# daniabib/ComfyUI_ProPainter_Nodes

Hardware: NVIDIA H100
Metric: inpainted frames/sec at 640x360, 80-frame subvideo (higher is better)
Workload: dtype f16

## Files before the change

### comfyui_propainter_nodes_b200/csrc/conv_epilogue.cuh

```cuda
#pragma once
#include "conv_igemm.cuh"
#include "wgmma_ops.cuh"

namespace ppconv {

template <int ACT, bool ACC = false>
__device__ __forceinline__ void act16_t(float (&v)[16], float slope) {
#pragma unroll
  for (int i = 0; i < 16; ++i) {
    if (ACT == PP_ACT_RELU) v[i] = fmaxf(v[i], 0.f);
    else if (ACT == PP_ACT_LRELU) v[i] = v[i] > 0.f ? v[i] : v[i] * slope;
    else if (ACT == PP_ACT_SIGMOID) v[i] = ppx::sigmoidf_(v[i]);
    else if (ACT == PP_ACT_TANH) v[i] = ACC ? ppx::tanh_acc(v[i]) : tanhf(v[i]);
    else if (ACT == PP_ACT_GELU) v[i] = ppx::gelu_erf(v[i]);
  }
}
template <bool ACC = false>
__device__ __forceinline__ void act16(float (&v)[16], int act, float slope) {
  switch (act) {
    case PP_ACT_RELU: act16_t<PP_ACT_RELU, ACC>(v, slope); break;
    case PP_ACT_LRELU: act16_t<PP_ACT_LRELU, ACC>(v, slope); break;
    case PP_ACT_SIGMOID: act16_t<PP_ACT_SIGMOID, ACC>(v, slope); break;
    case PP_ACT_TANH: act16_t<PP_ACT_TANH, ACC>(v, slope); break;
    case PP_ACT_GELU: act16_t<PP_ACT_GELU, ACC>(v, slope); break;
    default: break;
  }
}

__device__ __forceinline__ void load16(const __half* src, int nvalid, bool vec, float (&r)[16]) {
  if (vec && nvalid == 16) {
    const uint4 a = reinterpret_cast<const uint4*>(src)[0], b = reinterpret_cast<const uint4*>(src)[1];
    const __half2* ha = reinterpret_cast<const __half2*>(&a);
    const __half2* hb = reinterpret_cast<const __half2*>(&b);
#pragma unroll
    for (int i = 0; i < 4; ++i) {
      const float2 fa = __half22float2(ha[i]), fb = __half22float2(hb[i]);
      r[2 * i] = fa.x; r[2 * i + 1] = fa.y; r[8 + 2 * i] = fb.x; r[8 + 2 * i + 1] = fb.y;
    }
  } else {
#pragma unroll
    for (int i = 0; i < 16; ++i) r[i] = i < nvalid ? __half2float(src[i]) : 0.f;
  }
}
__device__ __forceinline__ void store16(__half* dst, int nvalid, bool vec, const float (&v)[16]) {
  if (vec && nvalid == 16) {
    __align__(16) __half2 h[8];
#pragma unroll
    for (int i = 0; i < 8; ++i) h[i] = __floats2half2_rn(v[2 * i], v[2 * i + 1]);
    reinterpret_cast<uint4*>(dst)[0] = reinterpret_cast<uint4*>(h)[0];
    reinterpret_cast<uint4*>(dst)[1] = reinterpret_cast<uint4*>(h)[1];
  } else {
#pragma unroll
    for (int i = 0; i < 16; ++i)
      if (i < nvalid) dst[i] = __float2half_rn(v[i]);
  }
}

__device__ __forceinline__ void unpack16(const uint4& a, const uint4& b, float (&r)[16]) {
  const __half2* ha = reinterpret_cast<const __half2*>(&a);
  const __half2* hb = reinterpret_cast<const __half2*>(&b);
#pragma unroll
  for (int i = 0; i < 4; ++i) {
    const float2 fa = __half22float2(ha[i]), fb = __half22float2(hb[i]);
    r[2 * i] = fa.x; r[2 * i + 1] = fa.y; r[8 + 2 * i] = fb.x; r[8 + 2 * i + 1] = fb.y;
  }
}

struct EpiAux {
  uint4 a0[2], a1[2];
  bool have;
};
__device__ __forceinline__ void conv_epilogue_prefetch16(const PPConvParams& p, long long mrow, int ng0, int epi, bool vec,
                                                         EpiAux& x) {
  x.have = false;
  if (!vec || p.Cout_g - ng0 < 16) return;
  const __half* s0 = nullptr;
  const __half* s1 = nullptr;
  if (epi == PP_EPI_STD) {
    if (p.aux0 != nullptr) s0 = p.aux0 + mrow * p.aux0_cstride + p.aux0_coff + ng0;
  } else if (epi == PP_EPI_GRU_ZR) {
    const int half_c = p.Cout_g >> 1;
    if (ng0 >= half_c) s0 = p.aux0 + mrow * p.aux0_cstride + p.aux0_coff + (ng0 - half_c);
  } else {
    s0 = p.aux0 + mrow * p.aux0_cstride + p.aux0_coff + ng0;
    s1 = p.aux1 + mrow * p.aux1_cstride + p.aux1_coff + ng0;
  }
  if (s0 == nullptr) return;
  x.have = true;
  x.a0[0] = reinterpret_cast<const uint4*>(s0)[0];
  x.a0[1] = reinterpret_cast<const uint4*>(s0)[1];
  if (s1 != nullptr) {
    x.a1[0] = reinterpret_cast<const uint4*>(s1)[0];
    x.a1[1] = reinterpret_cast<const uint4*>(s1)[1];
  }
}

__device__ __forceinline__ void conv_epilogue16(const PPConvParams& p, const uint32_t (&raw)[16], long long mrow, int g,
                                                int ng0, int epi, bool vec, const EpiAux* pre = nullptr,
                                                uint4* sm0 = nullptr, uint4* sm1 = nullptr) {
    const int nvalid = min(16, p.Cout_g - ng0);
    float v[16];
#pragma unroll
    for (int i = 0; i < 16; ++i) v[i] = __uint_as_float(raw[i]);
    if (p.bias != nullptr) {
      const float* bp = p.bias + g * p.Cout_g + ng0;
      if (vec && nvalid == 16) {
#pragma unroll
        for (int i = 0; i < 4; ++i) {
          const float4 b4 = __ldg(reinterpret_cast<const float4*>(bp) + i);
          v[4 * i] += b4.x; v[4 * i + 1] += b4.y; v[4 * i + 2] += b4.z; v[4 * i + 3] += b4.w;
        }
      } else {
#pragma unroll
        for (int i = 0; i < 16; ++i)
          if (i < nvalid) v[i] += __ldg(bp + i);
      }
    }
    if (epi == PP_EPI_STD) {
      act16(v, p.act1, p.slope);
      if (p.scale != 1.f) {
#pragma unroll
        for (int i = 0; i < 16; ++i) v[i] *= p.scale;
      }
      if (p.aux0 != nullptr) {
        float r[16];
        if (pre != nullptr && pre->have) unpack16(pre->a0[0], pre->a0[1], r);
        else load16(p.aux0 + mrow * p.aux0_cstride + p.aux0_coff + ng0, nvalid, vec, r);
#pragma unroll
        for (int i = 0; i < 16; ++i) v[i] += r[i];
      }
      act16(v, p.act2, p.slope);
      const long long o = mrow * p.out_cstride + p.out_coff + (long long)g * p.out_gstep + ng0;
      if (p.out_fp32) {
        float* dst = reinterpret_cast<float*>(p.out) + o;
        if (vec && nvalid == 16) {
#pragma unroll
          for (int i = 0; i < 4; ++i)
            reinterpret_cast<float4*>(dst)[i] = make_float4(v[4 * i], v[4 * i + 1], v[4 * i + 2], v[4 * i + 3]);
        } else {
#pragma unroll
          for (int i = 0; i < 16; ++i)
            if (i < nvalid) dst[i] = v[i];
        }
      } else if (sm0 != nullptr) {
        __align__(16) __half2 h[8];
#pragma unroll
        for (int i = 0; i < 8; ++i) h[i] = __floats2half2_rn(v[2 * i], v[2 * i + 1]);
        *sm0 = reinterpret_cast<uint4*>(h)[0];
        *sm1 = reinterpret_cast<uint4*>(h)[1];
      } else {
        store16(reinterpret_cast<__half*>(p.out) + o, nvalid, vec, v);
      }
    } else if (epi == PP_EPI_GRU_ZR) {
      const int half_c = p.Cout_g >> 1;
      act16_t<PP_ACT_SIGMOID>(v, 0.f);
      if (ng0 < half_c) {
        store16(reinterpret_cast<__half*>(p.out) + mrow * p.out_cstride + p.out_coff + ng0, nvalid, vec, v);
      } else {
        const int c = ng0 - half_c;
        float h[16];
        if (pre != nullptr && pre->have) unpack16(pre->a0[0], pre->a0[1], h);
        else load16(p.aux0 + mrow * p.aux0_cstride + p.aux0_coff + c, nvalid, vec, h);
#pragma unroll
        for (int i = 0; i < 16; ++i) v[i] *= h[i];
        store16(p.out2 + mrow * p.out2_cstride + p.out2_coff + c, nvalid, vec, v);
      }
    } else {
      float h[16], z[16];
      if (pre != nullptr && pre->have) {
        unpack16(pre->a0[0], pre->a0[1], h);
        unpack16(pre->a1[0], pre->a1[1], z);
      } else {
        load16(p.aux0 + mrow * p.aux0_cstride + p.aux0_coff + ng0, nvalid, vec, h);
        load16(p.aux1 + mrow * p.aux1_cstride + p.aux1_coff + ng0, nvalid, vec, z);
      }
      act16_t<PP_ACT_TANH>(v, 0.f);
#pragma unroll
      for (int i = 0; i < 16; ++i) v[i] = (1.f - z[i]) * h[i] + z[i] * v[i];
      store16(reinterpret_cast<__half*>(p.out) + mrow * p.out_cstride + p.out_coff + ng0, nvalid, vec, v);
    }
}

__device__ __forceinline__ float tf32_rna(float x) {
  uint32_t r;
  asm("cvt.rna.tf32.f32 %0, %1;" : "=r"(r) : "f"(x));
  return __uint_as_float(r);
}
__device__ __forceinline__ void load16_split(const float* src, int lo, int nvalid, bool vec, float (&r)[16]) {
  if (vec && nvalid == 16) {
#pragma unroll
    for (int i = 0; i < 4; ++i) {
      const float4 h = reinterpret_cast<const float4*>(src)[i], l = reinterpret_cast<const float4*>(src + lo)[i];
      r[4 * i] = h.x + l.x; r[4 * i + 1] = h.y + l.y; r[4 * i + 2] = h.z + l.z; r[4 * i + 3] = h.w + l.w;
    }
  } else {
#pragma unroll
    for (int i = 0; i < 16; ++i) r[i] = i < nvalid ? src[i] + src[lo + i] : 0.f;
  }
}
__device__ __forceinline__ void store16_split(float* dst, int lo, int nvalid, bool vec, const float (&v)[16]) {
  float h[16], l[16];
#pragma unroll
  for (int i = 0; i < 16; ++i) { h[i] = tf32_rna(v[i]); l[i] = v[i] - h[i]; }
  if (vec && nvalid == 16) {
#pragma unroll
    for (int i = 0; i < 4; ++i) {
      reinterpret_cast<float4*>(dst)[i] = make_float4(h[4 * i], h[4 * i + 1], h[4 * i + 2], h[4 * i + 3]);
      reinterpret_cast<float4*>(dst + lo)[i] = make_float4(l[4 * i], l[4 * i + 1], l[4 * i + 2], l[4 * i + 3]);
    }
  } else {
#pragma unroll
    for (int i = 0; i < 16; ++i)
      if (i < nvalid) { dst[i] = h[i]; dst[lo + i] = l[i]; }
  }
}

__device__ __forceinline__ void conv_epilogue16_split(const PPConvParams& p, const float (&acc)[16], long long mrow, int g,
                                                      int ng0, bool vec) {
  const int nvalid = min(16, p.Cout_g - ng0);
  float v[16];
#pragma unroll
  for (int i = 0; i < 16; ++i) v[i] = acc[i];
  if (p.bias != nullptr) {
    const float* bp = p.bias + g * p.Cout_g + ng0;
#pragma unroll
    for (int i = 0; i < 16; ++i)
      if (i < nvalid) v[i] += __ldg(bp + i);
  }
  const float* aux0 = reinterpret_cast<const float*>(p.aux0);
  const float* aux1 = reinterpret_cast<const float*>(p.aux1);
  float* out = reinterpret_cast<float*>(p.out);
  if (p.epi == PP_EPI_STD) {
    act16<true>(v, p.act1, p.slope);
    if (p.scale != 1.f) {
#pragma unroll
      for (int i = 0; i < 16; ++i) v[i] *= p.scale;
    }
    if (aux0 != nullptr) {
      float r[16];
      load16_split(aux0 + mrow * p.aux0_cstride + p.aux0_coff + ng0, p.aux0_lo, nvalid, vec, r);
#pragma unroll
      for (int i = 0; i < 16; ++i) v[i] += r[i];
    }
    act16<true>(v, p.act2, p.slope);
    float* dst = out + mrow * p.out_cstride + p.out_coff + (long long)g * p.out_gstep + ng0;
    if (p.out_fp32) {
      if (vec && nvalid == 16) {
#pragma unroll
        for (int i = 0; i < 4; ++i)
          reinterpret_cast<float4*>(dst)[i] = make_float4(v[4 * i], v[4 * i + 1], v[4 * i + 2], v[4 * i + 3]);
      } else {
#pragma unroll
        for (int i = 0; i < 16; ++i)
          if (i < nvalid) dst[i] = v[i];
      }
    } else {
      store16_split(dst, p.out_lo, nvalid, vec, v);
    }
  } else if (p.epi == PP_EPI_GRU_ZR) {
    const int half_c = p.Cout_g >> 1;
    act16_t<PP_ACT_SIGMOID, true>(v, 0.f);
    if (ng0 < half_c) {
      store16_split(out + mrow * p.out_cstride + p.out_coff + ng0, p.out_lo, nvalid, vec, v);
    } else {
      const int c = ng0 - half_c;
      float h[16];
      load16_split(aux0 + mrow * p.aux0_cstride + p.aux0_coff + c, p.aux0_lo, nvalid, vec, h);
#pragma unroll
      for (int i = 0; i < 16; ++i) v[i] *= h[i];
      store16_split(reinterpret_cast<float*>(p.out2) + mrow * p.out2_cstride + p.out2_coff + c, p.out2_lo, nvalid, vec, v);
    }
  } else {
    float h[16], z[16];
    load16_split(aux0 + mrow * p.aux0_cstride + p.aux0_coff + ng0, p.aux0_lo, nvalid, vec, h);
    load16_split(aux1 + mrow * p.aux1_cstride + p.aux1_coff + ng0, p.aux1_lo, nvalid, vec, z);
    act16_t<PP_ACT_TANH, true>(v, 0.f);
#pragma unroll
    for (int i = 0; i < 16; ++i) v[i] = (1.f - z[i]) * h[i] + z[i] * v[i];
    store16_split(out + mrow * p.out_cstride + p.out_coff + ng0, p.out_lo, nvalid, vec, v);
  }
}

constexpr int STG_LD = 40;
constexpr int STG_BYTES = 64 * STG_LD * 4;

template <int N, class Emit>
__device__ __forceinline__ void drain_acc(const float (&acc)[N / 2], float* stg, int t128, int bar_id, Emit&& emit) {
  const int wrow = 16 * (t128 >> 5) + ((t128 & 31) >> 2), wcol = 2 * (t128 & 3);
#pragma unroll 1
  for (int c0 = 0; c0 < N; c0 += 32) {
#pragma unroll
    for (int cc = 0; cc < N; cc += 32) {
      if (cc == c0) {
#pragma unroll
        for (int j = 0; j < 4; ++j) {
          if (cc + 8 * j < N) {
            const int i = (cc / 8 + j) * 4;
            *reinterpret_cast<float2*>(stg + wrow * STG_LD + 8 * j + wcol) = make_float2(acc[i], acc[i + 1]);
            *reinterpret_cast<float2*>(stg + (wrow + 8) * STG_LD + 8 * j + wcol) = make_float2(acc[i + 2], acc[i + 3]);
          }
        }
      }
    }
    ppx::named_bar(bar_id, 128);
    const int c = c0 + 16 * (t128 & 1);
    if (c < N) emit(stg + (t128 >> 1) * STG_LD + 16 * (t128 & 1), t128 >> 1, c);
    ppx::named_bar(bar_id, 128);
  }
}

template <bool SPLIT = false>
__device__ __forceinline__ void epilogue_from_stage(const PPConvParams& p, const float* src, long long mrow, int g, int ng0,
                                                    uint4* sm0, uint4* sm1) {
  if constexpr (SPLIT) {
    float acc[16];
#pragma unroll
    for (int i = 0; i < 16; i += 4) {
      const float4 v = *reinterpret_cast<const float4*>(src + i);
      acc[i] = v.x; acc[i + 1] = v.y; acc[i + 2] = v.z; acc[i + 3] = v.w;
    }
    conv_epilogue16_split(p, acc, mrow, g, ng0, p.vec_ok != 0);
  } else {
    uint32_t raw[16];
#pragma unroll
    for (int i = 0; i < 16; i += 4) {
      const float4 v = *reinterpret_cast<const float4*>(src + i);
      raw[i] = __float_as_uint(v.x); raw[i + 1] = __float_as_uint(v.y);
      raw[i + 2] = __float_as_uint(v.z); raw[i + 3] = __float_as_uint(v.w);
    }
    conv_epilogue16(p, raw, mrow, g, ng0, p.epi, p.vec_ok != 0, nullptr, sm0, sm1);
  }
}

template <int V>
struct IntC { static constexpr int value = V; };
template <int MAX_N, class F>
__device__ __forceinline__ void with_tile_width(int bn, F&& f) {
  switch (bn) {
    case 16: f(IntC<16>{}); break;
    case 32: f(IntC<32>{}); break;
    case 48: f(IntC<48>{}); break;
    case 64: f(IntC<64>{}); break;
    case 80: f(IntC<80>{}); break;
    case 96: f(IntC<96>{}); break;
    case 112: f(IntC<112>{}); break;
    case 128: f(IntC<128>{}); break;
    default:
      if constexpr (MAX_N > 128) {
        switch (bn) {
          case 144: f(IntC<144>{}); break;
          case 160: f(IntC<160>{}); break;
          case 176: f(IntC<176>{}); break;
          case 192: f(IntC<192>{}); break;
          case 208: f(IntC<208>{}); break;
          case 224: f(IntC<224>{}); break;
          case 240: f(IntC<240>{}); break;
          case 256: f(IntC<256>{}); break;
          default: __trap();
        }
      } else {
        __trap();
      }
  }
}

}
```

### comfyui_propainter_nodes_b200/csrc/conv_halo.cu

```cuda
#include <cuda.h>
#include <stdlib.h>
#include <string.h>

#include <memory>

#include "conv_epilogue.cuh"
#include "conv_igemm.cuh"
#include "dcn_sample.cuh"

namespace {

constexpr int NUM_THREADS = 384;
constexpr int NUM_EPI_THREADS = 256;
constexpr int WARP_A = 8, WARP_B = 9;
constexpr int MAX_SA = 4, MAX_SB = 8;
constexpr int SMEM_BUDGET = 186 * 1024;

struct HaloParams {
  PPConvParams c;
  CUtensorMap tmap[PP_MAX_SEGS];
  int MT;
  int BW, BH;
  int tiles_x, tiles_y, n_tiles;
  int a_stage_bytes, b_stage_bytes, SA, SB;
  int tps;
  int chunks;
  int flat;
  int n_img;
  int sub_bytes;
  int debug;
  int tstore;
  int out_stage_bytes;
  CUtensorMap tmap_out;
};

__device__ __forceinline__ void tma_load_4d(uint32_t dst, const void* tmap, int c0, int c1, int c2, int c3, uint64_t* bar) {
  asm volatile(
      "cp.async.bulk.tensor.4d.shared::cluster.global.mbarrier::complete_tx::bytes [%0], [%1, {%3, %4, %5, %6}], [%2];" ::"r"(dst),
      "l"(tmap), "r"(ppx::smem_u32(bar)), "r"(c0), "r"(c1), "r"(c2), "r"(c3)
      : "memory");
}

__device__ __forceinline__ void tma_store_2d(const void* tmap, uint32_t src, int c0, int c1) {
  asm volatile("cp.async.bulk.tensor.2d.global.shared::cta.bulk_group [%0, {%2, %3}], [%1];" ::"l"(tmap), "r"(src), "r"(c0), "r"(c1)
               : "memory");
}

struct TileCoord {
  int n_idx, tx, ty, img, g;
};
__device__ __forceinline__ TileCoord decode_tile(const HaloParams& h, int tile) {
  TileCoord t;
  t.n_idx = tile % h.n_tiles;
  int r = tile / h.n_tiles;
  t.tx = r % h.tiles_x; r /= h.tiles_x;
  t.ty = r % h.tiles_y; r /= h.tiles_y;
  t.img = r % h.n_img;
  t.g = r / h.n_img;
  return t;
}

__host__ __device__ inline int halo_total_tiles(const HaloParams& h) {
  return h.n_tiles * h.tiles_x * h.tiles_y * h.n_img * h.c.groups;
}

struct Ring {
  int s;
  uint32_t ph;
};

struct HaloSmem {
  uint8_t* a;
  uint8_t* b;
  int SA, SB, a_stage_bytes, b_stage_bytes;
  uint64_t *a_full, *a_empty, *b_full, *b_empty;
  uint64_t* spare;
  uint8_t* out_stg;
  float* acc_stg;
  int bytes;
};

__host__ __device__ inline HaloSmem halo_smem(uint8_t* base, int SA, int a_stage_bytes, int SB, int b_stage_bytes,
                                              int out_bytes) {
  const int b_off = SA * a_stage_bytes, bar_off = b_off + SB * b_stage_bytes, out_off = bar_off + 1024;
  const int acc_off = out_off + out_bytes;
  HaloSmem m;
  m.SA = SA; m.SB = SB; m.a_stage_bytes = a_stage_bytes; m.b_stage_bytes = b_stage_bytes;
  m.a = base;
  m.b = base + b_off;
  m.a_full = reinterpret_cast<uint64_t*>(base + bar_off);
  m.a_empty = m.a_full + MAX_SA;
  m.b_full = m.a_empty + MAX_SA;
  m.b_empty = m.b_full + MAX_SB;
  m.spare = m.b_empty + MAX_SB;
  m.out_stg = out_bytes > 0 ? base + out_off : nullptr;
  m.acc_stg = reinterpret_cast<float*>(base + acc_off);
  m.bytes = 1024 + acc_off + 2 * ppconv::STG_BYTES;
  return m;
}

__device__ __forceinline__ uint8_t* halo_smem_base() {
  extern __shared__ uint8_t smem_raw[];
  const uint32_t raw_addr = ppx::smem_u32(smem_raw);
  return smem_raw + (((raw_addr + 1023u) & ~1023u) - raw_addr);
}

__host__ __device__ constexpr int halo_max_tps(int bn) { return 128 / bn > 1 ? 128 / bn : 1; }

template <int BN, int MB, bool TF32>
__device__ __forceinline__ void halo_tap(float (&acc)[MB][BN / 2], uint64_t (&adesc)[MB], uint64_t& bdesc, uint32_t& accum,
                                         int& kx, int kw, uint32_t step_x, uint32_t step_row, uint32_t tap16) {
#pragma unroll
  for (int k = 0; k < 4; ++k)
#pragma unroll
    for (int b = 0; b < MB; ++b) {
      if constexpr (TF32) ppx::wgmma_tf32<BN>(acc[b], adesc[b] + 2 * k, bdesc + 2 * k, (accum | k) != 0 ? 1u : 0u);
      else ppx::wgmma_f16<BN>(acc[b], adesc[b] + 2 * k, bdesc + 2 * k, (accum | k) != 0 ? 1u : 0u);
    }
  accum = 1u;
  bdesc += tap16;
  const uint32_t step = ++kx == kw ? step_row : step_x;
  if (kx == kw) kx = 0;
#pragma unroll
  for (int b = 0; b < MB; ++b) adesc[b] += step;
}

template <int BN, int MB, int NT, bool TF32>
__device__ __forceinline__ void halo_tap_group(int tn, float (&acc)[MB][BN / 2], uint64_t (&adesc)[MB], uint64_t bdesc,
                                               uint32_t& accum, int& kx, int kw, uint32_t step_x, uint32_t step_row,
                                               uint32_t tap16) {
  using namespace ppx;
  if constexpr (NT == 0) {
    wgmma_fence();
    for (int tt = 0; tt < tn; ++tt) halo_tap<BN, MB, TF32>(acc, adesc, bdesc, accum, kx, kw, step_x, step_row, tap16);
    wgmma_commit();
  } else {
    if constexpr (NT > 1) {
      if (tn < NT) {
        halo_tap_group<BN, MB, NT - 1, TF32>(tn, acc, adesc, bdesc, accum, kx, kw, step_x, step_row, tap16);
        return;
      }
    }
    wgmma_fence();
#pragma unroll
    for (int tt = 0; tt < NT; ++tt) halo_tap<BN, MB, TF32>(acc, adesc, bdesc, accum, kx, kw, step_x, step_row, tap16);
    wgmma_commit();
  }
}

template <int BN, int MB, int NT, bool TF32 = false>
__device__ __forceinline__ void halo_tile(const HaloParams& h, int tile, const HaloSmem& m, Ring& ra, Ring& rb, float* stg,
                                          int wg, int t128) {
  using namespace ppx;
  const PPConvParams& p = h.c;
  const int taps = p.kh * p.kw;
  const TileCoord t = decode_tile(h, tile);
  const int n0 = t.n_idx * p.BN;
  const int bnt = min(p.BN, p.Cout_g_pad - n0);
  const uint32_t sbo = h.flat ? 1024u : (uint32_t)h.BW * 128;
  const uint32_t step_x = (uint32_t)p.dw * 8;
  const uint32_t step_row = (uint32_t)(p.dh * h.BW - (p.kw - 1) * p.dw) * 8;
  const uint32_t tap16 = (uint32_t)p.BN * 8;
  const int kw = p.kw;
  uint32_t aoff[MB];
#pragma unroll
  for (int b = 0; b < MB; ++b) aoff[b] = MB == 2 ? wg * h.sub_bytes + b * 8 * sbo : wg * 8 * sbo;
  float acc[MB][BN / 2];
  uint32_t accum = 0;
  int pend_a = -1, pend_b = -1;
  for (int c = 0; c < h.chunks; ++c) {
    mbar_wait(&m.a_full[ra.s], ra.ph);
    uint64_t adesc[MB];
#pragma unroll
    for (int b = 0; b < MB; ++b) adesc[b] = gmma_desc_sw128_kmajor(smem_u32(m.a + ra.s * m.a_stage_bytes) + aoff[b], sbo);
    int kx = 0;
    for (int tap0 = 0; tap0 < taps; tap0 += h.tps) {
      mbar_wait(&m.b_full[rb.s], rb.ph);
      const uint64_t bdesc = gmma_desc_sw128_kmajor(smem_u32(m.b + rb.s * m.b_stage_bytes));
      halo_tap_group<BN, MB, NT, TF32>(min(h.tps, taps - tap0), acc, adesc, bdesc, accum, kx, kw, step_x, step_row, tap16);
      wgmma_wait<1>();
      if (pend_b >= 0) mbar_arrive(&m.b_empty[pend_b]);
      if (pend_a >= 0) mbar_arrive(&m.a_empty[pend_a]);
      pend_b = rb.s;
      pend_a = tap0 + h.tps >= taps ? ra.s : -1;
      if (++rb.s == m.SB) { rb.s = 0; rb.ph ^= 1; }
    }
    if (++ra.s == m.SA) { ra.s = 0; ra.ph ^= 1; }
  }
  wgmma_wait<0>();
#pragma unroll
  for (int b = 0; b < MB; ++b) wgmma_fence_acc(acc[b]);
  if (pend_b >= 0) mbar_arrive(&m.b_empty[pend_b]);
  if (pend_a >= 0) mbar_arrive(&m.a_empty[pend_a]);

  const bool skip = (h.debug & 1) != 0;
  const int bar_id = 2 + (MB == 2 ? wg : 0), bar_n = MB == 2 ? 128 : 256;
  const bool issuer = t128 == 0 && (MB == 2 || wg == 0);
  uint8_t* so = h.tstore ? m.out_stg + (MB == 2 ? wg : 0) * h.out_stage_bytes : nullptr;
  if (so != nullptr) {
    if (issuer) asm volatile("cp.async.bulk.wait_group.read 0;" ::: "memory");
    named_bar(bar_id, bar_n);
  }
#pragma unroll
  for (int b = 0; b < MB; ++b) {
    const int sub = MB == 2 ? wg : 0, rbase = MB == 2 ? 64 * b : 64 * wg;
    ppconv::drain_acc<BN>(acc[b], stg, t128, 4 + wg, [&](const float* src, int r64, int cc) {
      const int r = rbase + r64;
      bool mvalid;
      long long mrow;
      if (h.flat) {
        mrow = ((long long)t.tx * h.MT + sub) * 128 + r;
        mvalid = mrow < p.M_total;
      } else {
        const int oy = t.ty * 16 + (r >> 3), ox = t.tx * (8 * h.MT) + 8 * sub + (r & 7);
        mvalid = oy < p.OH && ox < p.OW;
        mrow = ((long long)t.img * p.OH + oy) * p.OW + ox;
      }
      if (!mvalid || skip || cc >= bnt || n0 + cc >= p.Cout_g) return;
      if (!TF32 && so != nullptr) {
        auto slot = [&](int u) {
          const int unit = ((cc & 63) >> 3) + u;
          return reinterpret_cast<uint4*>(so + (cc >> 6) * 16384 + r * 128 + ((unit ^ (r & 7)) << 4));
        };
        ppconv::epilogue_from_stage(p, src, mrow, t.g, n0 + cc, slot(0), slot(1));
      } else {
        ppconv::epilogue_from_stage<TF32>(p, src, mrow, t.g, n0 + cc, nullptr, nullptr);
      }
    });
  }
  if (so != nullptr) {
    fence_proxy_async();
    named_bar(bar_id, bar_n);
    if (issuer && !skip) {
      const int row0 = (int)(((long long)t.tx * h.MT + (MB == 2 ? wg : 0)) * 128);
      for (int pnl = 0; pnl * 64 < bnt; ++pnl)
        tma_store_2d(&h.tmap_out, smem_u32(so + pnl * 16384), n0 + pnl * 64, row0);
      asm volatile("cp.async.bulk.commit_group;" ::: "memory");
    }
  }
}

template <class F>
__device__ __forceinline__ void with_tile_shape(int mt, int bn, F&& f) {
  if (mt == 2) ppconv::with_tile_width<128>(bn, [&](auto n) { f(n, ppconv::IntC<2>{}); });
  else ppconv::with_tile_width<256>(bn, [&](auto n) { f(n, ppconv::IntC<1>{}); });
}

__device__ __forceinline__ void halo_smem_init_barriers(const HaloSmem& m) {
  using namespace ppx;
  for (int s = 0; s < m.SA; ++s) { mbar_init(&m.a_full[s], 1); mbar_init(&m.a_empty[s], NUM_EPI_THREADS); }
  for (int s = 0; s < m.SB; ++s) { mbar_init(&m.b_full[s], 1); mbar_init(&m.b_empty[s], NUM_EPI_THREADS); }
  mbar_fence_init();
}

__device__ __forceinline__ void halo_produce_patches(const HaloParams& h, const HaloSmem& m, Ring& r) {
  using namespace ppx;
  const PPConvParams& p = h.c;
  const int total_tiles = halo_total_tiles(h);
  const uint32_t bytes = (uint32_t)(h.BW * h.BH * 128);
  for (int tile = blockIdx.x; tile < total_tiles; tile += gridDim.x) {
    const TileCoord t = decode_tile(h, tile);
    const int x0 = h.flat ? t.tx * (128 * h.MT) : t.tx * (8 * h.MT) - p.pw, y0 = h.flat ? 0 : t.ty * 16 - p.ph;
    for (int c = 0; c < h.chunks; ++c) {
      const int ci = c * 64;
      int q = 0;
#pragma unroll
      for (int k = 1; k < PP_MAX_SEGS; ++k)
        if (k < p.nseg && ci >= p.seg[k].cbegin) q = k;
      const int ch0 = t.g * p.seg[q].gstep + (ci - p.seg[q].cbegin);
      mbar_wait(&m.a_empty[r.s], r.ph ^ 1);
      mbar_arrive_expect_tx(&m.a_full[r.s], bytes);
      tma_load_4d(smem_u32(m.a + r.s * m.a_stage_bytes), &h.tmap[q], ch0, x0, y0, t.img, &m.a_full[r.s]);
      if (++r.s == m.SA) { r.s = 0; r.ph ^= 1; }
    }
  }
}

__device__ __forceinline__ void halo_produce_weights(const HaloParams& h, const HaloSmem& m, Ring& r) {
  using namespace ppx;
  const PPConvParams& p = h.c;
  const int total_tiles = halo_total_tiles(h);
  const int taps = p.kh * p.kw;
  for (int tile = blockIdx.x; tile < total_tiles; tile += gridDim.x) {
    const TileCoord t = decode_tile(h, tile);
    const int n0 = t.n_idx * p.BN;
    const uint32_t bytes = (uint32_t)(min(p.BN, p.Cout_g_pad - n0) * 128);
    const __half* wbase = p.wpacked + ((long long)t.g * p.num_kc * p.Cout_g_pad + n0) * 64;
    for (int c = 0; c < h.chunks; ++c) {
      for (int tap0 = 0; tap0 < taps; tap0 += h.tps) {
        const int tn = min(h.tps, taps - tap0);
        mbar_wait(&m.b_empty[r.s], r.ph ^ 1);
        mbar_arrive_expect_tx(&m.b_full[r.s], bytes * (uint32_t)tn);
        for (int t = 0; t < tn; ++t) {
          const int kc = (tap0 + t) * h.chunks + c;
          bulk_g2s(smem_u32(m.b + r.s * m.b_stage_bytes + t * p.BN * 128), wbase + (long long)kc * p.Cout_g_pad * 64, bytes,
                   &m.b_full[r.s]);
        }
        if (++r.s == m.SB) { r.s = 0; r.ph ^= 1; }
      }
    }
  }
}

template <bool TF32>
__device__ __forceinline__ void halo_body(const HaloParams& h) {
  using namespace ppx;
  const HaloSmem m =
      halo_smem(halo_smem_base(), h.SA, h.a_stage_bytes, h.SB, h.b_stage_bytes, h.tstore ? h.MT * h.out_stage_bytes : 0);
  const int tid = threadIdx.x, warp = tid >> 5;
  if (tid == 0) halo_smem_init_barriers(m);
  __syncthreads();
  asm volatile("griddepcontrol.wait;" ::: "memory");
  asm volatile("griddepcontrol.launch_dependents;" ::: "memory");

  if (warp < 8) setmaxnreg_inc<232>();
  else setmaxnreg_dec<40>();
  if (warp < 8) {
    const int wg = tid >> 7, t128 = tid & 127;
    float* stg = m.acc_stg + wg * (ppconv::STG_BYTES / 4);
    Ring ra = {0, 0}, rb = {0, 0};
    const int total_tiles = halo_total_tiles(h);
    with_tile_shape(h.MT, h.c.BN, [&](auto bn, auto mb) {
      constexpr int BN = decltype(bn)::value;
      for (int tile = blockIdx.x; tile < total_tiles; tile += gridDim.x)
        halo_tile<BN, decltype(mb)::value, halo_max_tps(BN), TF32>(h, tile, m, ra, rb, stg, wg, t128);
    });
    if (h.tstore) asm volatile("cp.async.bulk.wait_group 0;" ::: "memory");
  } else if (warp == WARP_A) {
    if (elect_one()) {
      Ring r = {0, 0};
      halo_produce_patches(h, m, r);
    }
  } else if (warp == WARP_B) {
    if (elect_one()) {
      Ring r = {0, 0};
      halo_produce_weights(h, m, r);
    }
  }
}

__global__ void __launch_bounds__(NUM_THREADS, 1) conv_halo_kernel(const __grid_constant__ HaloParams h) {
  halo_body<false>(h);
}

__global__ void __launch_bounds__(NUM_THREADS, 1) conv_halo_tf32_kernel(const __grid_constant__ HaloParams h) {
  halo_body<true>(h);
}

constexpr int PROG_MAX_LAYERS = 10;
enum { PROG_CONV = 0, PROG_DCN = 1 };

struct ProgParams {
  int n_layers;
  int SA, SB, a_stage_bytes, b_stage_bytes;
  unsigned int* counter;
  unsigned int base;
  unsigned long long* ts;
  int kind[PROG_MAX_LAYERS];
  PPDcnArgs dcn[PROG_MAX_LAYERS];
  HaloParams layer[PROG_MAX_LAYERS];
};

__device__ __forceinline__ void prog_wait(const unsigned int* counter, unsigned int target) {
  unsigned int v, spins = 0;
  uint64_t t0 = 0;
  for (;;) {
    asm volatile("ld.acquire.gpu.global.u32 %0, [%1];" : "=r"(v) : "l"(counter) : "memory");
    if ((int)(v - target) >= 0) return;
    __nanosleep(64);
    if ((++spins & 0xFFFu) == 0) {
      uint64_t now;
      asm volatile("mov.u64 %0, %%globaltimer;" : "=l"(now));
      if (t0 == 0) t0 = now;
      else if (now - t0 > 2000000000ull) __trap();
    }
  }
}
__device__ __forceinline__ void fence_proxy_async_global() { asm volatile("fence.proxy.async.global;" ::: "memory"); }

__global__ void __launch_bounds__(NUM_THREADS, 1) conv_prog_kernel(const __grid_constant__ ProgParams P) {
  using namespace ppx;
  const HaloSmem m = halo_smem(halo_smem_base(), P.SA, P.a_stage_bytes, P.SB, P.b_stage_bytes, 0);
  uint64_t* layer_go = m.spare;

  const int tid = threadIdx.x, warp = tid >> 5;
  const unsigned int G = gridDim.x;
  if (tid == 0) {
    mbar_init(layer_go, 1);
    halo_smem_init_barriers(m);
  }
  __syncthreads();
  asm volatile("griddepcontrol.wait;" ::: "memory");
  asm volatile("griddepcontrol.launch_dependents;" ::: "memory");

  if (warp < 8) setmaxnreg_inc<232>();
  else setmaxnreg_dec<40>();
  if (warp < 8) {
    const int wg = tid >> 7, t128 = tid & 127;
    float* stg = m.acc_stg + wg * (ppconv::STG_BYTES / 4);
    Ring ra = {0, 0}, rb = {0, 0};
    for (int li = 0; li < P.n_layers; ++li) {
      mbar_wait(layer_go, (uint32_t)li & 1u);
      if (P.ts != nullptr && blockIdx.x == 0 && tid == 0) {
        unsigned long long now;
        asm volatile("mov.u64 %0, %%globaltimer;" : "=l"(now));
        P.ts[2 * li] = now;
      }
      if (P.kind[li] == PROG_DCN) {
        const PPDcnArgs& a = P.dcn[li];
        const unsigned per_img = (unsigned)(a.H * a.W * 144);
        const unsigned total = per_img * (unsigned)a.N;
        const unsigned stride = G * NUM_EPI_THREADS;
        for (unsigned idx = blockIdx.x * NUM_EPI_THREADS + tid; idx < total; idx += 4 * stride) {
#pragma unroll
          for (int u = 0; u < 4; ++u) {
            const unsigned i2 = idx + u * stride;
            if (i2 < total) {
              const unsigned n = i2 / per_img;
              if (a.C == 128) dcn_sample_item<8, true>(a, i2 - n * per_img, (int)n);
              else dcn_sample_item<16, true>(a, i2 - n * per_img, (int)n);
            }
          }
        }
      } else {
        const HaloParams& h = P.layer[li];
        const int total_tiles = halo_total_tiles(h);
        ppconv::with_tile_width<128>(h.c.BN, [&](auto bn) {
          for (int tile = blockIdx.x; tile < total_tiles; tile += G)
            halo_tile<decltype(bn)::value, 1, 0>(h, tile, m, ra, rb, stg, wg, t128);
        });
      }
      fence_proxy_async_global();
      asm volatile("bar.sync 1, %0;" ::"n"(NUM_EPI_THREADS) : "memory");
      if (tid == 0) {
        __threadfence();
        atomicAdd(P.counter, 1u);
        if (P.ts != nullptr && blockIdx.x == 0) {
          unsigned long long now;
          asm volatile("mov.u64 %0, %%globaltimer;" : "=l"(now));
          P.ts[2 * li + 1] = now;
        }
      }
    }
  } else if (warp == WARP_A) {
    if (elect_one()) {
      Ring r = {0, 0};
      for (int li = 0; li < P.n_layers; ++li) {
        if (li > 0) {
          prog_wait(P.counter, P.base + (unsigned int)li * G);
          fence_proxy_async_global();
        }
        mbar_arrive(layer_go);
        if (P.kind[li] == PROG_CONV) halo_produce_patches(P.layer[li], m, r);
      }
    }
  } else if (warp == WARP_B) {
    if (elect_one()) {
      Ring r = {0, 0};
      for (int li = 0; li < P.n_layers; ++li)
        if (P.kind[li] == PROG_CONV) halo_produce_weights(P.layer[li], m, r);
    }
  }
}

typedef CUresult (*EncodeTiledFn)(CUtensorMap*, CUtensorMapDataType, cuuint32_t, void*, const cuuint64_t*, const cuuint64_t*,
                                  const cuuint32_t*, const cuuint32_t*, CUtensorMapInterleave, CUtensorMapSwizzle,
                                  CUtensorMapL2promotion, CUtensorMapFloatOOBfill);

EncodeTiledFn encode_fn() {
  static EncodeTiledFn fn = nullptr;
  static bool tried = false;
  if (!tried) {
    tried = true;
    cudaDriverEntryPointQueryResult qr;
    void* ptr = nullptr;
    if (cudaGetDriverEntryPoint("cuTensorMapEncodeTiled", &ptr, cudaEnableDefault, &qr) == cudaSuccess &&
        qr == cudaDriverEntryPointSuccess)
      fn = reinterpret_cast<EncodeTiledFn>(ptr);
  }
  return fn;
}

}

int pp_conv_halo_eligible(const PPConvParams& p) {
  static int enabled = -1;
  if (enabled < 0) {
    const char* e = getenv("PP_CONV_HALO");
    enabled = (e == nullptr || atoi(e) != 0) ? 1 : 0;
  }
  if (!enabled) return 0;
  if (p.sh != 1 || p.sw != 1 || p.pad_replicate) return 0;
  const bool flat = p.kh * p.kw == 1;
  if (flat) {
    if (p.ph != 0 || p.pw != 0 || p.groups != 1) return 0;
  } else if (p.Cin % 64 != 0) {
    return 0;
  }
  for (int i = 0; i < p.nseg; ++i) {
    if (p.seg[i].cbegin % 64 != 0) return 0;
    if (p.seg[i].cend % 64 != 0 && !(flat && i == p.nseg - 1)) return 0;
  }
  if ((p.kw - 1) * p.dw + 16 > 256 || (p.kh - 1) * p.dh + 16 > 256) return 0;
  if ((long long)p.N * p.OH * p.OW < 128) return 0;
  return encode_fn() != nullptr ? 1 : 0;
}

namespace {

int halo_num_sms(int* out) {
  static int num_sms = 0;
  if (num_sms == 0) {
    int dev = 0;
    PP_CUDA_CHECK(cudaGetDevice(&dev));
    PP_CUDA_CHECK(cudaDeviceGetAttribute(&num_sms, cudaDevAttrMultiProcessorCount, dev));
    PP_CUDA_CHECK(cudaFuncSetAttribute(conv_halo_kernel, cudaFuncAttributeMaxDynamicSharedMemorySize, 224 * 1024));
    PP_CUDA_CHECK(cudaFuncSetAttribute(conv_halo_tf32_kernel, cudaFuncAttributeMaxDynamicSharedMemorySize, 224 * 1024));
    PP_CUDA_CHECK(cudaFuncSetAttribute(conv_prog_kernel, cudaFuncAttributeMaxDynamicSharedMemorySize, 224 * 1024));
  }
  *out = num_sms;
  return PP_OK;
}

bool halo_stages(int budget, int a_bytes, int b_bytes, int& sa, int& sb) {
  for (sa = 3; sa >= 2; --sa) {
    sb = (budget - sa * a_bytes) / b_bytes;
    if (sb >= 3) {
      if (sb > MAX_SB) sb = MAX_SB;
      return true;
    }
  }
  return false;
}

template <class Params>
int halo_launch(void (*kernel)(Params), const Params& params, int grid, int smem_bytes, cudaStream_t stream) {
  cudaLaunchConfig_t cfg;
  memset(&cfg, 0, sizeof(cfg));
  cfg.gridDim = dim3(grid);
  cfg.blockDim = dim3(NUM_THREADS);
  cfg.dynamicSmemBytes = smem_bytes;
  cfg.stream = stream;
  cudaLaunchAttribute attr[1];
  attr[0].id = cudaLaunchAttributeProgrammaticStreamSerialization;
  attr[0].val.programmaticStreamSerializationAllowed = 1;
  cfg.attrs = attr;
  cfg.numAttrs = 1;
  PP_CUDA_CHECK(cudaLaunchKernelEx(&cfg, kernel, params));
  PP_CUDA_CHECK(cudaGetLastError());
  return PP_OK;
}

int halo_configure(const PPConvParams& pin, HaloParams& h, bool one_wave) {
  h.c = pin;
  PPConvParams& p = h.c;
  int num_sms = 0;
  PP_TRY(halo_num_sms(&num_sms));
  const bool flat = p.kh * p.kw == 1;
  const int n_tiles0 = pp_ceil_div(p.Cout_g_pad, 128);
  int bn = pp_ceil_div(pp_ceil_div(p.Cout_g_pad, n_tiles0), 16) * 16;
  const int tiles_y = flat ? 1 : pp_ceil_div(p.OH, 16);
  auto tiles_x = [&](int mt) { return flat ? (int)pp_ceil_div64(p.M_total, 128 * mt) : pp_ceil_div(p.OW, 8 * mt); };
  const int n_img = flat ? 1 : p.N;
  auto count = [&](int mt, int bn_) {
    return (long long)pp_ceil_div(p.Cout_g_pad, bn_) * tiles_x(mt) * tiles_y * n_img * p.groups;
  };
  int mt = count(2, bn) < num_sms ? 1 : 2;
  while (count(mt, bn) < num_sms && bn >= 64 && bn % 32 == 0) bn /= 2;
  if (one_wave) {
    mt = 1;
    for (int nt = 8; nt >= 1; --nt) {
      const int b = pp_ceil_div(pp_ceil_div(p.Cout_g_pad, nt), 16) * 16;
      if (b > 128 || b < 16) continue;
      if (count(1, b) <= num_sms) { mt = 1; bn = b; break; }
    }
  }
  p.BN = bn;
  h.MT = mt;
  h.flat = flat ? 1 : 0;
  h.n_img = n_img;
  h.BW = flat ? 128 * mt : 8 * mt + (p.kw - 1) * p.dw;
  h.BH = flat ? 1 : 16 + (p.kh - 1) * p.dh;
  h.sub_bytes = flat ? 128 * 128 : 8 * 128;
  h.tiles_x = tiles_x(mt);
  h.tiles_y = tiles_y;
  h.n_tiles = pp_ceil_div(p.Cout_g_pad, bn);
  h.chunks = pp_ceil_div(p.Cin, 64);
  h.a_stage_bytes = pp_ceil_div(h.BW * h.BH * 128, 1024) * 1024;
  h.tps = min(halo_max_tps(bn), p.kh * p.kw);
  h.b_stage_bytes = h.tps * bn * 128;
  h.tstore = 0;
  h.out_stage_bytes = 0;
  if (!one_wave && flat && !p.split && p.epi == PP_EPI_STD && !p.out_fp32 && p.groups == 1 && p.out_gstep == 0 && bn % 64 == 0 &&
      p.vec_ok && h.chunks <= 16 && p.out_cstride % 8 == 0 && p.out_coff % 8 == 0 &&
      (reinterpret_cast<uintptr_t>(p.out) & 15) == 0) {
    h.tstore = 1;
    h.out_stage_bytes = (bn / 64) * 16384;
  }
  int sa = 0, sb = 0;
  if (h.tstore && !halo_stages(SMEM_BUDGET - mt * h.out_stage_bytes, h.a_stage_bytes, h.b_stage_bytes, sa, sb)) {
    h.tstore = 0;
    h.out_stage_bytes = 0;
  }
  const int budget = SMEM_BUDGET - mt * h.out_stage_bytes;
  PP_REQUIRE(halo_stages(budget, h.a_stage_bytes, h.b_stage_bytes, sa, sb), "conv_halo: patch %dx%d does not fit shared memory",
             h.BW, h.BH);
  if (sa == 3 && sb == MAX_SB && (budget - 4 * h.a_stage_bytes) / h.b_stage_bytes >= MAX_SB) sa = 4;
  h.SA = sa; h.SB = sb;
  if (h.tstore) {
    cuuint64_t dims[2] = {(cuuint64_t)p.Cout_g, (cuuint64_t)p.M_total};
    cuuint64_t strides[1] = {(cuuint64_t)p.out_cstride * 2};
    cuuint32_t box[2] = {64, 128};
    cuuint32_t es[2] = {1, 1};
    EncodeTiledFn enc_o = encode_fn();
    PP_REQUIRE(enc_o != nullptr, "conv_halo: cuTensorMapEncodeTiled is not available");
    const CUresult r = enc_o(&h.tmap_out, CU_TENSOR_MAP_DATA_TYPE_FLOAT16, 2, reinterpret_cast<__half*>(p.out) + p.out_coff, dims,
                             strides, box, es, CU_TENSOR_MAP_INTERLEAVE_NONE, CU_TENSOR_MAP_SWIZZLE_128B,
                             CU_TENSOR_MAP_L2_PROMOTION_L2_128B, CU_TENSOR_MAP_FLOAT_OOB_FILL_NONE);
    PP_REQUIRE(r == CUDA_SUCCESS, "conv_halo: cuTensorMapEncodeTiled (output) failed (%d)", (int)r);
  }
  { const char* e = getenv("PP_CONV_NOEPI"); h.debug = (e != nullptr && atoi(e) != 0) ? 1 : 0; }
  const long long total_tiles = count(mt, bn);
  PP_REQUIRE(total_tiles < (1LL << 31), "conv_halo: too many tiles");

  EncodeTiledFn enc = encode_fn();
  PP_REQUIRE(enc != nullptr, "conv_halo: cuTensorMapEncodeTiled is not available");
  for (int i = 0; i < p.nseg; ++i) {
    const PPConvSeg& s = p.seg[i];
    const cuuint64_t cacc = (cuuint64_t)(p.groups - 1) * s.gstep + (s.cvalid > 0 ? s.cvalid : s.cend - s.cbegin);
    cuuint64_t dims[4] = {cacc, (cuuint64_t)p.W, (cuuint64_t)p.H, (cuuint64_t)p.N};
    cuuint64_t strides[3] = {(cuuint64_t)s.cstride * 2, (cuuint64_t)p.W * s.cstride * 2, (cuuint64_t)p.H * p.W * s.cstride * 2};
    cuuint32_t box[4] = {64, (cuuint32_t)h.BW, (cuuint32_t)h.BH, 1};
    if (flat) {
      dims[1] = (cuuint64_t)p.M_total; dims[2] = 1; dims[3] = 1;
      strides[1] = strides[2] = (cuuint64_t)p.M_total * s.cstride * 2;
    }
    cuuint32_t es[4] = {1, 1, 1, 1};
    const CUresult r = enc(&h.tmap[i], CU_TENSOR_MAP_DATA_TYPE_FLOAT16, 4, const_cast<__half*>(s.ptr + s.coff), dims, strides, box,
                           es, CU_TENSOR_MAP_INTERLEAVE_NONE, CU_TENSOR_MAP_SWIZZLE_128B,
                           CU_TENSOR_MAP_L2_PROMOTION_L2_128B, CU_TENSOR_MAP_FLOAT_OOB_FILL_NONE);
    PP_REQUIRE(r == CUDA_SUCCESS, "conv_halo: cuTensorMapEncodeTiled failed (%d) for segment %d (cstride=%d W=%d H=%d N=%d)",
               (int)r, i, s.cstride, p.W, p.H, p.N);
  }
  return PP_OK;
}

}

int pp_launch_conv_halo(const PPConvParams& pin, cudaStream_t stream) {
  HaloParams h;
  PP_TRY(halo_configure(pin, h, false));
  int num_sms = 0;
  PP_TRY(halo_num_sms(&num_sms));
  const int smem = halo_smem(nullptr, h.SA, h.a_stage_bytes, h.SB, h.b_stage_bytes, h.tstore ? h.MT * h.out_stage_bytes : 0).bytes;
  return halo_launch(h.c.split ? conv_halo_tf32_kernel : conv_halo_kernel, h, min(halo_total_tiles(h), num_sms), smem, stream);
}

namespace {
thread_local PPProgRecorder* g_recorder = nullptr;
}

struct PPProgRecorder {
  ProgParams prog;
  double flops = 0.0;
  int n_conv = 0;
};

bool pp_prog_recording() { return g_recorder != nullptr; }

int pp_prog_begin() {
  PP_REQUIRE(g_recorder == nullptr, "conv program: already recording");
  g_recorder = new PPProgRecorder();
  memset(&g_recorder->prog, 0, sizeof(ProgParams));
  return PP_OK;
}

void pp_prog_abort() {
  delete g_recorder;
  g_recorder = nullptr;
}

int pp_prog_record_conv(const PPConvParams& p) {
  PPProgRecorder* r = g_recorder;
  PP_REQUIRE(r != nullptr, "conv program: not recording");
  PP_REQUIRE(r->prog.n_layers < PROG_MAX_LAYERS, "conv program: more than %d layers", PROG_MAX_LAYERS);
  PP_REQUIRE(pp_conv_halo_eligible(p), "conv program: layer is not a stride-1 TMA halo-kernel convolution");
  PP_REQUIRE(!p.split, "conv program: split-tf32 layers are not supported");
  const int li = r->prog.n_layers;
  PP_TRY(halo_configure(p, r->prog.layer[li], true));
  PP_REQUIRE(r->prog.layer[li].MT == 1 && r->prog.layer[li].c.BN <= 128, "conv program: layer tile %d x %d columns",
             r->prog.layer[li].MT, r->prog.layer[li].c.BN);
  r->prog.kind[li] = PROG_CONV;
  r->prog.n_layers++;
  r->n_conv++;
  return PP_OK;
}

int pp_prog_record_dcn(const PPDcnArgs& a) {
  PPProgRecorder* r = g_recorder;
  PP_REQUIRE(r != nullptr, "conv program: not recording");
  PP_REQUIRE(r->prog.n_layers < PROG_MAX_LAYERS, "conv program: more than %d layers", PROG_MAX_LAYERS);
  const int li = r->prog.n_layers;
  r->prog.kind[li] = PROG_DCN;
  r->prog.dcn[li] = a;
  r->prog.n_layers++;
  return PP_OK;
}

int pp_prog_end(unsigned int* counter, unsigned int* arrivals, cudaStream_t stream) {
  PPProgRecorder* r = g_recorder;
  PP_REQUIRE(r != nullptr, "conv program: not recording");
  g_recorder = nullptr;
  std::unique_ptr<PPProgRecorder> guard(r);
  ProgParams& P = r->prog;
  if (P.n_layers == 0) return PP_OK;
  int num_sms = 0;
  PP_TRY(halo_num_sms(&num_sms));
  int a_max = 1024, b_max = 2048;
  for (int i = 0; i < P.n_layers; ++i)
    if (P.kind[i] == PROG_CONV) {
      if (P.layer[i].a_stage_bytes > a_max) a_max = P.layer[i].a_stage_bytes;
      if (P.layer[i].b_stage_bytes > b_max) b_max = P.layer[i].b_stage_bytes;
    }
  int sa = 0, sb = 0;
  PP_REQUIRE(halo_stages(SMEM_BUDGET, a_max, b_max, sa, sb), "conv program: stages do not fit shared memory (A %d B, B %d B)",
             a_max, b_max);
  P.SA = sa; P.SB = sb; P.a_stage_bytes = a_max; P.b_stage_bytes = b_max;
  P.counter = counter;
  P.base = *arrivals;
  static int ts_mode = -1, ts_printed = 0;
  static unsigned long long* ts_dev = nullptr;
  if (ts_mode < 0) {
    const char* e = getenv("PP_PROG_TS");
    ts_mode = (e != nullptr && atoi(e) != 0) ? atoi(e) : 0;
    if (ts_mode) PP_CUDA_CHECK(cudaMalloc(&ts_dev, 2 * PROG_MAX_LAYERS * sizeof(unsigned long long)));
  }
  P.ts = (ts_mode && ts_printed < ts_mode) ? ts_dev : nullptr;
  const int grid = num_sms;
  *arrivals += (unsigned int)(P.n_layers * grid);
  PP_TRY(halo_launch(conv_prog_kernel, P, grid, halo_smem(nullptr, sa, a_max, sb, b_max, 0).bytes, stream));
  if (P.ts != nullptr) {
    unsigned long long h[2 * PROG_MAX_LAYERS];
    PP_CUDA_CHECK(cudaStreamSynchronize(stream));
    PP_CUDA_CHECK(cudaMemcpy(h, ts_dev, sizeof(h), cudaMemcpyDeviceToHost));
    ++ts_printed;
    fprintf(stderr, "[prog %d] %d layers:", ts_printed, P.n_layers);
    for (int i = 0; i < P.n_layers; ++i) {
      const HaloParams& L = P.layer[i];
      if (P.kind[i] == PROG_CONV)
        fprintf(stderr, " | conv K=%d N=%d bn=%d mt=%d tiles=%d: %.1f us (gap %.1f)", L.c.K_total, L.c.Cout_g, L.c.BN, L.MT,
                halo_total_tiles(L), (h[2 * i + 1] - h[2 * i]) / 1e3, i ? (h[2 * i] - h[2 * i - 1]) / 1e3 : 0.0);
      else
        fprintf(stderr, " | dcn: %.1f us (gap %.1f)", (h[2 * i + 1] - h[2 * i]) / 1e3, i ? (h[2 * i] - h[2 * i - 1]) / 1e3 : 0.0);
    }
    fprintf(stderr, " | total %.1f us\n", (h[2 * P.n_layers - 1] - h[0]) / 1e3);
  }
  return PP_OK;
}
```

Before: 153.9.

## Specialize persistent conv program to fixed tile widths with unrolled tap groups

The multi-layer persistent conv program now instantiates only three tile widths (32, 64, 224) and picks among them by minimizing waves times columns, instead of searching for the widest tile that fits one wave. The tile loop uses a compile-time tap-group size with unrolled wgmma batches instead of the runtime-count path, and the epilogue mode and TMA-store path are fixed at compile time. The aim is to cut code size and register pressure, reduce runtime branching, and allow wider tiles that reuse the A halo across more output channels. In exchange, layers whose configuration does not fit these widths are rejected, and 224-wide tiles may raise register use.

```diff
diff --git a/comfyui_propainter_nodes_b200/csrc/conv_epilogue.cuh b/comfyui_propainter_nodes_b200/csrc/conv_epilogue.cuh
--- a/comfyui_propainter_nodes_b200/csrc/conv_epilogue.cuh
+++ b/comfyui_propainter_nodes_b200/csrc/conv_epilogue.cuh
@@ -309,7 +309,7 @@
   }
 }
 
-template <bool SPLIT = false>
+template <bool SPLIT = false, int EPI = -1>
 __device__ __forceinline__ void epilogue_from_stage(const PPConvParams& p, const float* src, long long mrow, int g, int ng0,
                                                     uint4* sm0, uint4* sm1) {
   if constexpr (SPLIT) {
@@ -328,7 +328,7 @@
       raw[i] = __float_as_uint(v.x); raw[i + 1] = __float_as_uint(v.y);
       raw[i + 2] = __float_as_uint(v.z); raw[i + 3] = __float_as_uint(v.w);
     }
-    conv_epilogue16(p, raw, mrow, g, ng0, p.epi, p.vec_ok != 0, nullptr, sm0, sm1);
+    conv_epilogue16(p, raw, mrow, g, ng0, EPI >= 0 ? EPI : p.epi, p.vec_ok != 0, nullptr, sm0, sm1);
   }
 }
 
diff --git a/comfyui_propainter_nodes_b200/csrc/conv_halo.cu b/comfyui_propainter_nodes_b200/csrc/conv_halo.cu
--- a/comfyui_propainter_nodes_b200/csrc/conv_halo.cu
+++ b/comfyui_propainter_nodes_b200/csrc/conv_halo.cu
@@ -130,25 +130,19 @@
                                                uint32_t& accum, int& kx, int kw, uint32_t step_x, uint32_t step_row,
                                                uint32_t tap16) {
   using namespace ppx;
-  if constexpr (NT == 0) {
-    wgmma_fence();
-    for (int tt = 0; tt < tn; ++tt) halo_tap<BN, MB, TF32>(acc, adesc, bdesc, accum, kx, kw, step_x, step_row, tap16);
-    wgmma_commit();
-  } else {
-    if constexpr (NT > 1) {
-      if (tn < NT) {
-        halo_tap_group<BN, MB, NT - 1, TF32>(tn, acc, adesc, bdesc, accum, kx, kw, step_x, step_row, tap16);
-        return;
-      }
-    }
-    wgmma_fence();
-#pragma unroll
-    for (int tt = 0; tt < NT; ++tt) halo_tap<BN, MB, TF32>(acc, adesc, bdesc, accum, kx, kw, step_x, step_row, tap16);
-    wgmma_commit();
-  }
-}
-
-template <int BN, int MB, int NT, bool TF32 = false>
+  if constexpr (NT > 1) {
+    if (tn < NT) {
+      halo_tap_group<BN, MB, NT - 1, TF32>(tn, acc, adesc, bdesc, accum, kx, kw, step_x, step_row, tap16);
+      return;
+    }
+  }
+  wgmma_fence();
+#pragma unroll
+  for (int tt = 0; tt < NT; ++tt) halo_tap<BN, MB, TF32>(acc, adesc, bdesc, accum, kx, kw, step_x, step_row, tap16);
+  wgmma_commit();
+}
+
+template <int BN, int MB, int NT, bool TF32 = false, bool PROG = false>
 __device__ __forceinline__ void halo_tile(const HaloParams& h, int tile, const HaloSmem& m, Ring& ra, Ring& rb, float* stg,
                                           int wg, int t128) {
   using namespace ppx;
@@ -196,7 +190,7 @@
   const bool skip = (h.debug & 1) != 0;
   const int bar_id = 2 + (MB == 2 ? wg : 0), bar_n = MB == 2 ? 128 : 256;
   const bool issuer = t128 == 0 && (MB == 2 || wg == 0);
-  uint8_t* so = h.tstore ? m.out_stg + (MB == 2 ? wg : 0) * h.out_stage_bytes : nullptr;
+  uint8_t* so = !PROG && h.tstore ? m.out_stg + (MB == 2 ? wg : 0) * h.out_stage_bytes : nullptr;
   if (so != nullptr) {
     if (issuer) asm volatile("cp.async.bulk.wait_group.read 0;" ::: "memory");
     named_bar(bar_id, bar_n);
@@ -224,7 +218,7 @@
         };
         ppconv::epilogue_from_stage(p, src, mrow, t.g, n0 + cc, slot(0), slot(1));
       } else {
-        ppconv::epilogue_from_stage<TF32>(p, src, mrow, t.g, n0 + cc, nullptr, nullptr);
+        ppconv::epilogue_from_stage<TF32, PROG ? PP_EPI_STD : -1>(p, src, mrow, t.g, n0 + cc, nullptr, nullptr);
       }
     });
   }
@@ -350,6 +344,19 @@
 constexpr int PROG_MAX_LAYERS = 10;
 enum { PROG_CONV = 0, PROG_DCN = 1 };
 
+constexpr int PROG_WIDTHS[] = {32, 64, 224};
+
+template <class F>
+__device__ __forceinline__ void with_prog_width(int bn, F&& f) {
+  static_assert(sizeof(PROG_WIDTHS) == 3 * sizeof(int), "with_prog_width: one case per PROG_WIDTHS entry");
+  switch (bn) {
+    case PROG_WIDTHS[0]: f(ppconv::IntC<PROG_WIDTHS[0]>{}); break;
+    case PROG_WIDTHS[1]: f(ppconv::IntC<PROG_WIDTHS[1]>{}); break;
+    case PROG_WIDTHS[2]: f(ppconv::IntC<PROG_WIDTHS[2]>{}); break;
+    default: __trap();
+  }
+}
+
 struct ProgParams {
   int n_layers;
   int SA, SB, a_stage_bytes, b_stage_bytes;
@@ -425,9 +432,10 @@
       } else {
         const HaloParams& h = P.layer[li];
         const int total_tiles = halo_total_tiles(h);
-        ppconv::with_tile_width<128>(h.c.BN, [&](auto bn) {
+        with_prog_width(h.c.BN, [&](auto bn) {
+          constexpr int BN = decltype(bn)::value;
           for (int tile = blockIdx.x; tile < total_tiles; tile += G)
-            halo_tile<decltype(bn)::value, 1, 0>(h, tile, m, ra, rb, stg, wg, t128);
+            halo_tile<BN, 1, halo_max_tps(BN), false, true>(h, tile, m, ra, rb, stg, wg, t128);
         });
       }
       fence_proxy_async_global();
@@ -569,10 +577,14 @@
   while (count(mt, bn) < num_sms && bn >= 64 && bn % 32 == 0) bn /= 2;
   if (one_wave) {
     mt = 1;
-    for (int nt = 8; nt >= 1; --nt) {
-      const int b = pp_ceil_div(pp_ceil_div(p.Cout_g_pad, nt), 16) * 16;
-      if (b > 128 || b < 16) continue;
-      if (count(1, b) <= num_sms) { mt = 1; bn = b; break; }
+    long long best_cols = -1, best_waves = 0;
+    for (const int b : PROG_WIDTHS) {
+      const long long waves = (count(1, b) + num_sms - 1) / num_sms;
+      if (best_cols < 0 || waves * b < best_cols || (waves * b == best_cols && waves < best_waves)) {
+        best_cols = waves * b;
+        best_waves = waves;
+        bn = b;
+      }
     }
   }
   p.BN = bn;
@@ -686,10 +698,12 @@
   PP_REQUIRE(r->prog.n_layers < PROG_MAX_LAYERS, "conv program: more than %d layers", PROG_MAX_LAYERS);
   PP_REQUIRE(pp_conv_halo_eligible(p), "conv program: layer is not a stride-1 TMA halo-kernel convolution");
   PP_REQUIRE(!p.split, "conv program: split-tf32 layers are not supported");
+  PP_REQUIRE(p.epi == PP_EPI_STD, "conv program: only the plain epilogue (bias, activations, residual) is compiled in");
   const int li = r->prog.n_layers;
   PP_TRY(halo_configure(p, r->prog.layer[li], true));
-  PP_REQUIRE(r->prog.layer[li].MT == 1 && r->prog.layer[li].c.BN <= 128, "conv program: layer tile %d x %d columns",
-             r->prog.layer[li].MT, r->prog.layer[li].c.BN);
+  const HaloParams& h = r->prog.layer[li];
+  PP_REQUIRE(h.MT == 1 && !h.tstore && (h.c.BN == PROG_WIDTHS[0] || h.c.BN == PROG_WIDTHS[1] || h.c.BN == PROG_WIDTHS[2]),
+             "conv program: layer tile %d x %d columns is not instantiated", h.MT, h.c.BN);
   r->prog.kind[li] = PROG_CONV;
   r->prog.n_layers++;
   r->n_conv++;
```

Result: faster. 158.8, median of 6 (+3.2%).
